# cestpasphoto/alpha-zero-general

Hardware: AMD Instinct MI355X
Metric: self-play env-steps/sec @ numMCTSSims=800, Splendor-2p (higher is better)
Workload: dtype f64

## Files before the change

alpha-zero-general_amd/csrc/game_splendor.hip.h:

```cpp
#pragma once
#include "azg_common.hip.h"
#include "splendor_tables.h"

namespace azg {

template <int NP>
struct SplendorDev {
    static constexpr bool STOCHASTIC = false;
    static constexpr bool RANDOM_SYM = false;
    static constexpr int P = NP;
    static constexpr int NN = NP + 1;
    static constexpr int ROWS = 32 + 10 * NP + NP * NP;
    static constexpr int COLS = 7;
    static constexpr int S = ROWS * COLS;
    static constexpr int SP = RoundUp16<S>::value;
    static constexpr int A = 81;
    static constexpr int AW = 2;
    static constexpr int R_NOBLES = 31, R_GEMS = 32 + NP, R_PNOB = 32 + 2 * NP, R_PCARDS = 32 + 3 * NP + NP * NP,
                         R_RES = 32 + 4 * NP + NP * NP;
    static constexpr int GOLD = 5, PTS = 6;
    static constexpr int MAX_MOVES = 62 * NP;

    __device__ static __forceinline__ const int8_t* row(const int8_t* st, int r) { return st + r * COLS; }
    __device__ static __forceinline__ int8_t* row(int8_t* st, int r) { return st + r * COLS; }
    __device__ static __forceinline__ int sum5(const int8_t* r) { return r[0] + r[1] + r[2] + r[3] + r[4]; }
    __device__ static __forceinline__ int sum7(const int8_t* r) { return sum5(r) + r[5] + r[6]; }

    __device__ static __forceinline__ int missing(const int8_t* cost, const int8_t* gems, const int8_t* cards) {
        int s = 0;
#pragma unroll
        for (int c = 0; c < 5; c++) {
            int8_t d = (int8_t)((int8_t)(cost[c] - gems[c]) - cards[c]);
            s += d > 0 ? d : 0;
        }
        return s;
    }

    __device__ static __forceinline__ void valid_mask(const int8_t* st, int player, uint64_t* mask_lds) {
        const int l = lane_id();
        const int8_t* bankp = row(st, 0);
        const int8_t* gemsp = row(st, R_GEMS + player);
        const int8_t* cardsp = row(st, R_PCARDS + player);
        const int8_t* lastres = row(st, R_RES + 6 * player + 5);
        int bank[5], gems[7], cards[5];
#pragma unroll
        for (int c = 0; c < 5; c++) { bank[c] = bankp[c]; cards[c] = cardsp[c]; }
#pragma unroll
        for (int c = 0; c < 7; c++) gems[c] = gemsp[c];
        const bool empty_slot = sum5(lastres) == 0;
        const int r = l < 12 ? 1 + 2 * l : l < 24 ? 1 + 2 * (l - 12) : l < 27 ? 25 + 2 * (l - 24)
                    : l < 30 ? R_RES + 6 * player + 2 * (l - 27) : 0;
        const int8_t* cr = row(st, r);
        int cost[5];
#pragma unroll
        for (int c = 0; c < 5; c++) cost[c] = cr[c];
        int gsum = 0;
#pragma unroll
        for (int c = 0; c < 7; c++) gsum += gems[c];
        int miss = 0, csum = 0;
#pragma unroll
        for (int c = 0; c < 5; c++) {
            const int8_t d = (int8_t)((int8_t)(cost[c] - gems[c]) - cards[c]);
            miss += d > 0 ? d : 0;
            csum += cost[c];
        }
        const bool nz = csum != 0;
        const bool ok_buy = miss <= gems[GOLD] && nz;
        const bool ok_res = empty_slot && nz;
        constexpr uint32_t g3[5] = SPL_GEMS3_COL_INIT, g2[5] = SPL_GEMS2_COL_INIT;
        const int i3 = (l - 30) & 31;
        const int ig = (l >= 60 ? l - 60 : l + 4) & 15;
        bool ok3 = true, okg = true;
        int k3 = 0;
#pragma unroll
        for (int c = 0; c < 5; c++) {
            const int t3 = (int)((g3[c] >> i3) & 1u), t2 = (int)((g2[c] >> ig) & 1u);
            ok3 = ok3 && ((int8_t)(bank[c] - t3) >= 0);
            okg = okg && ((int8_t)(gems[c] - t2) >= 0);
            k3 += t3;
        }
        ok3 = ok3 && (gsum + k3 <= 10);
        const int cs = l - 55, cg = l - 11;
        int bank_cs = bank[0], gems_cg = gems[0];
#pragma unroll
        for (int c = 1; c < 5; c++) { bank_cs = cs == c ? bank[c] : bank_cs; gems_cg = cg == c ? gems[c] : gems_cg; }
        const bool ok_same = bank_cs >= 4 && gsum + 2 <= 10;
        const bool v0 = l < 12 ? ok_buy : l < 27 ? ok_res : l < 30 ? ok_buy : l < 55 ? ok3 : l < 60 ? ok_same : okg;
        const bool v1 = l < 11 ? okg : l < 16 ? gems_cg >= 2 : l == 16;
        const uint64_t m0 = __ballot(v0);
        const uint64_t m1 = __ballot(v1);
        if (l == 0) { mask_lds[0] = m0; mask_lds[1] = m1; }
    }

    __device__ static bool get_deck_card(int8_t* st, int tier, long long seed, Rng& rng, int8_t* card14) {
        int8_t* cnt = row(st, 25 + 2 * tier);
        int8_t* bits = row(st, 26 + 2 * tier);
        int total = sum5(cnt);
        if (total == 0) return false;
        int color = 0, card_index = 0;
        if (seed == 0) {
            double u = rng.u01(), acc = 0.0;
            int k = 0;
            for (; k < 5; k++) { acc += (double)cnt[k] / (double)total; if (acc > u) break; }
            if (k >= 5) { for (k = 4; k > 0 && cnt[k] == 0; k--) {} }
            color = k;
            uint32_t b = (uint8_t)bits[color];
            int nb = __popc(b);
            double u2 = rng.u01();
            acc = 0.0;
            int idx = -1, last = 0;
            for (int i = 0; i < 8; i++) {
                int set = (b >> (7 - i)) & 1;
                if (set) last = i;
                acc += (double)set / (double)nb;
                if (acc > u2) { idx = i; break; }
            }
            card_index = idx < 0 ? last : idx;
        } else {
            int n = 0;
            long long seedv = 0, pw = 1;
            for (int c = 0; c < 5; c++) {
                uint32_t b = (uint8_t)bits[c];
                n += __popc(b);
                seedv += (long long)b * pw;
                pw *= 32;
            }
            long long x = 4594591LL * (seed + seedv);
            long long r = x % n;
            if (r < 0) r += n;
            int rem = (int)r;
            for (int c = 0; c < 5; c++) {
                uint32_t b = (uint8_t)bits[c];
                int pc = __popc(b);
                if (rem < pc) {
                    color = c;
                    for (int i = 0; i < 8; i++)
                        if ((b >> (7 - i)) & 1) { if (rem == 0) { card_index = i; break; } rem--; }
                    break;
                }
                rem -= pc;
            }
        }
        uint32_t b = (uint8_t)bits[color];
        b &= ~(0x80u >> card_index);
        bits[color] = (int8_t)(uint8_t)b;
        cnt[color] -= 1;
#pragma unroll
        for (int i = 0; i < 14; i++) card14[i] = SPL_CARDS[tier][color][card_index][i];
        return true;
    }

    __device__ static void fill_new_card(int8_t* st, int tier, int index, long long seed, Rng& rng) {
        int8_t* dst = row(st, 1 + 8 * tier + 2 * index);
        int8_t card[14];
        bool got = get_deck_card(st, tier, seed, rng, card);
#pragma unroll
        for (int i = 0; i < 14; i++) dst[i] = got ? card[i] : (int8_t)0;
    }

    static constexpr int SPW = SP / 4, NW = (SPW + 63) / 64;
    struct SW {
        uint32_t w[NW];
        __device__ __forceinline__ void load(const int8_t* st) {
#pragma unroll
            for (int k = 0; k < NW; k++) { const int i = lane_id() + 64 * k; w[k] = i < SPW ? ((const uint32_t*)st)[i] : 0u; }
        }
        __device__ __forceinline__ void store(int8_t* st) const {
#pragma unroll
            for (int k = 0; k < NW; k++) { const int i = lane_id() + 64 * k; if (i < SPW) ((uint32_t*)st)[i] = w[k]; }
        }
        __device__ __forceinline__ uint32_t rd(int d) const {
            uint32_t v = (uint32_t)__builtin_amdgcn_readlane((int)w[0], d & 63);
#pragma unroll
            for (int k = 1; k < NW; k++) {
                const uint32_t vk = (uint32_t)__builtin_amdgcn_readlane((int)w[k], d & 63);
                v = (d >> 6) == k ? vk : v;
            }
            return v;
        }
        __device__ __forceinline__ void wr(int d, uint32_t v) {
#pragma unroll
            for (int k = 0; k < NW; k++) w[k] = (lane_id() + 64 * k == d) ? v : w[k];
        }
        __device__ __forceinline__ uint64_t row(int r) const {
            const int o = 7 * r, d = o >> 2, sh = (o & 3) * 8;
            uint64_t v = (((uint64_t)rd(d + 1) << 32) | rd(d)) >> sh;
            if (sh > 8) v |= (uint64_t)rd(d + 2) << (64 - sh);
            return v & 0x00FFFFFFFFFFFFFFull;
        }
        __device__ __forceinline__ void set_row(int r, uint64_t v) {
            const int o = 7 * r, d = o >> 2, sh = (o & 3) * 8;
            const uint64_t m = 0x00FFFFFFFFFFFFFFull, M = m << sh, V = (v & m) << sh;
            wr(d, (rd(d) & ~(uint32_t)M) | (uint32_t)V);
            wr(d + 1, (rd(d + 1) & ~(uint32_t)(M >> 32)) | (uint32_t)(V >> 32));
            if (sh > 8) wr(d + 2, (rd(d + 2) & ~(uint32_t)(m >> (64 - sh))) | (uint32_t)((v & m) >> (64 - sh)));
        }
    };
    __device__ static __forceinline__ int B(uint64_t row, int c) { return (int)(int8_t)(uint8_t)(row >> (8 * c)); }
    __device__ static __forceinline__ int UB(uint64_t row, int c) { return (int)(uint8_t)(row >> (8 * c)); }
    __device__ static __forceinline__ void SETB(uint64_t& row, int c, int v) {
        row = (row & ~(0xFFull << (8 * c))) | ((uint64_t)(uint8_t)v << (8 * c));
    }
    __device__ static __forceinline__ int rsum5(uint64_t r) { return B(r, 0) + B(r, 1) + B(r, 2) + B(r, 3) + B(r, 4); }
    __device__ static __forceinline__ int rsum7(uint64_t r) { return rsum5(r) + B(r, 5) + B(r, 6); }

    __device__ static __forceinline__ uint32_t small_mod(uint32_t v, uint32_t n, float rn) {
        const uint32_t q = (uint32_t)((float)v * rn);
        int r = (int)(v - q * n);
        r = r < 0 ? r + (int)n : r;
        r = r >= (int)n ? r - (int)n : r;
        return (uint32_t)r;
    }
    __device__ static __forceinline__ int draw_mod(long long b, int n) {
        const float rn = 1.0f / (float)n;
        const bool neg = b < 0;
        const uint64_t ub = neg ? (uint64_t)(-b) : (uint64_t)b;
        uint32_t mb = 0;
#pragma unroll
        for (int k = 3; k >= 0; k--) mb = small_mod(mb * 65536u + (uint32_t)((ub >> (16 * k)) & 0xFFFFu), (uint32_t)n, rn);
        uint32_t ma = small_mod(70u, (uint32_t)n, rn);
        ma = small_mod(ma * 65536u + 7071u, (uint32_t)n, rn);
        uint32_t r = small_mod(ma * mb, (uint32_t)n, rn);
        if (neg && r) r = (uint32_t)n - r;
        return (int)r;
    }

    __device__ static __forceinline__ bool draw_card(SW& s, int tier, long long seed, Rng& rng, int* color_o, int* idx_o) {
        uint64_t cnt = s.row(25 + 2 * tier), bits = s.row(26 + 2 * tier);
        const int total = rsum5(cnt);
        if (total == 0) return false;
        int color = 0, card_index = 0;
        if (seed == 0) {
            const double u = rng.u01();
            double acc = 0.0;
            int k = 0;
            for (; k < 5; k++) { acc += (double)B(cnt, k) / (double)total; if (acc > u) break; }
            if (k >= 5) { for (k = 4; k > 0 && B(cnt, k) == 0; k--) {} }
            color = k;
            const uint32_t b = (uint32_t)UB(bits, color);
            const int nb = __popc(b);
            const double u2 = rng.u01();
            acc = 0.0;
            int idx = -1, last = 0;
            for (int i = 0; i < 8; i++) {
                const int set = (b >> (7 - i)) & 1;
                if (set) last = i;
                acc += (double)set / (double)nb;
                if (acc > u2) { idx = i; break; }
            }
            card_index = idx < 0 ? last : idx;
        } else {
            int n = 0;
            long long seedv = 0, pw = 1;
#pragma unroll
            for (int c = 0; c < 5; c++) {
                const uint32_t b = (uint32_t)UB(bits, c);
                n += __popc(b);
                seedv += (long long)b * pw;
                pw *= 32;
            }
            int rem = draw_mod(seed + seedv, n);
            for (int c = 0; c < 5; c++) {
                const uint32_t b = (uint32_t)UB(bits, c);
                const int pc = __popc(b);
                if (rem < pc) {
                    color = c;
                    for (int i = 0; i < 8; i++)
                        if ((b >> (7 - i)) & 1) { if (rem == 0) { card_index = i; break; } rem--; }
                    break;
                }
                rem -= pc;
            }
        }
        SETB(bits, color, (int)((uint32_t)UB(bits, color) & ~(0x80u >> card_index)));
        SETB(cnt, color, B(cnt, color) - 1);
        s.set_row(25 + 2 * tier, cnt);
        s.set_row(26 + 2 * tier, bits);
        *color_o = color; *idx_o = card_index;
        return true;
    }

    __device__ static __forceinline__ void buy_card(SW& s, uint64_t& bank, uint64_t& gems, uint64_t c0, uint64_t c1, int player) {
        uint64_t cards = s.row(R_PCARDS + player);
        int miss = 0;
#pragma unroll
        for (int c = 0; c < 5; c++) {
            const int8_t d = (int8_t)((int8_t)(B(c0, c) - B(gems, c)) - B(cards, c));
            miss += d > 0 ? d : 0;
        }
#pragma unroll
        for (int c = 0; c < 5; c++) {
            int8_t need = (int8_t)(B(c0, c) - B(cards, c));
            need = need < 0 ? (int8_t)0 : need;
            const int8_t g = (int8_t)B(gems, c);
            const int8_t paid = need < g ? need : g;
            SETB(gems, c, g - paid);
            SETB(bank, c, B(bank, c) + paid);
        }
        SETB(gems, GOLD, B(gems, GOLD) - miss);
        SETB(bank, GOLD, B(bank, GOLD) + miss);
#pragma unroll
        for (int c = 0; c < COLS; c++) SETB(cards, c, B(cards, c) + B(c1, c));
        s.set_row(R_PCARDS + player, cards);
        for (int i = 0; i < NN; i++) {
            const uint64_t noble = s.row(R_NOBLES + i);
            if (rsum5(noble) <= 0) continue;
            bool ok = true;
#pragma unroll
            for (int c = 0; c < 5; c++) ok = ok && B(cards, c) >= B(noble, c);
            if (ok) {
                s.set_row(R_PNOB + NN * player + i, noble);
                s.set_row(R_NOBLES + i, 0ull);
            }
        }
    }

    __device__ static __forceinline__ int gc_age(const int8_t* st) { return get_round(st); }

    __device__ static __forceinline__ bool move_uses_seed(int move) { return move < 27; }
    static constexpr int SEED_ACTIONS = 27;

    __device__ static int wave_make_move(int8_t* st, int move, int player, long long seed, Rng& rng) {
        move = uni_i32(move); player = uni_i32(player);
        seed = (long long)(((uint64_t)uni_u32((uint32_t)((uint64_t)seed >> 32)) << 32) | uni_u32((uint32_t)seed));
        const int l = lane_id();
        SW s;
        s.load(st);
        uint64_t bank = s.row(0), gems = s.row(R_GEMS + player);
        const int res = R_RES + 6 * player;
        int fill_row = -1, fill_tier = 0, fill_color = 0, fill_idx = 0;
        bool fill_got = false;
        int copy_src = -1, copy_dst = 0;
        int shift_i = -1;
        if (move < 12) {
            buy_card(s, bank, gems, s.row(1 + 2 * move), s.row(2 + 2 * move), player);
            fill_tier = move >> 2;
            fill_got = draw_card(s, fill_tier, seed, rng, &fill_color, &fill_idx);
            fill_row = 1 + 2 * move;
        } else if (move < 27) {
            const int i = move - 12;
            int slot = 2;
            for (int k = 2; k >= 0; k--) if (rsum5(s.row(res + 2 * k)) == 0) slot = k;
            if (i < 12) {
                copy_src = 1 + 2 * i; copy_dst = res + 2 * slot;
                fill_tier = i >> 2;
                fill_got = draw_card(s, fill_tier, seed, rng, &fill_color, &fill_idx);
                fill_row = 1 + 2 * i;
            } else {
                fill_tier = i - 12;
                fill_got = draw_card(s, fill_tier, seed, rng, &fill_color, &fill_idx);
                if (fill_got) fill_row = res + 2 * slot;
            }
            if (B(bank, GOLD) > 0 && rsum7(gems) <= 9) { SETB(gems, GOLD, B(gems, GOLD) + 1); SETB(bank, GOLD, B(bank, GOLD) - 1); }
        } else if (move < 30) {
            const int i = move - 27;
            buy_card(s, bank, gems, s.row(res + 2 * i), s.row(res + 2 * i + 1), player);
            shift_i = i;
        } else if (move < 80) {
            constexpr uint32_t g3[5] = SPL_GEMS3_COL_INIT, g2[5] = SPL_GEMS2_COL_INIT;
            const bool take = move < 60;
            const int i = take ? move - 30 : move - 60, nd = take ? 25 : 15;
#pragma unroll
            for (int c = 0; c < 5; c++) {
                const int k = i < nd ? (int)(((take ? g3[c] : g2[c]) >> (i & 31)) & 1u) : (c == i - nd ? 2 : 0);
                SETB(bank, c, take ? B(bank, c) - k : B(bank, c) + k);
                SETB(gems, c, take ? B(gems, c) + k : B(gems, c) - k);
            }
        }
        SETB(bank, PTS, B(bank, PTS) + 1);
        s.set_row(0, bank);
        s.set_row(R_GEMS + player, gems);
        s.store(st);
        wave_sync();
        if (copy_src >= 0 && l < 14) st[copy_dst * COLS + l] = st[copy_src * COLS + l];
        if (fill_row >= 0 && l < 14)
            st[fill_row * COLS + l] = fill_got ? SPL_CARDS[fill_tier][fill_color][fill_idx][l] : (int8_t)0;
        if (shift_i >= 0 && l < 6 * COLS) {
            const int lo = 2 * shift_i * COLS;
            const int8_t v = (l >= lo && l < 4 * COLS) ? st[res * COLS + l + 2 * COLS] : (int8_t)0;
            if (l >= lo) st[res * COLS + l] = v;
        }
        wave_sync();
        return (player + 1) % NP;
    }

    __device__ static __forceinline__ int get_round(const int8_t* st) { return (uint8_t)st[PTS]; }

    __device__ static int get_score(const int8_t* st, int p) {
        int s = row(st, R_PCARDS + p)[PTS];
#pragma unroll
        for (int i = 0; i < NN; i++) s += row(st, R_PNOB + NN * p + i)[PTS];
        return s;
    }

    __device__ static bool game_ended(const int8_t* st, int next_player, float* out , uint64_t* mask_scratch) {
        (void)next_player; (void)mask_scratch;
        int round = get_round(st);
#pragma unroll
        for (int p = 0; p < NP; p++) out[p] = 0.f;
        if (round % NP != 0) return false;
        float sc[NP];
        float mx = -1e30f;
#pragma unroll
        for (int p = 0; p < NP; p++) { sc[p] = (float)get_score(st, p); mx = sc[p] > mx ? sc[p] : mx; }
        if (!(mx >= 15.f || round >= MAX_MOVES)) return false;
        int cnt = 0;
#pragma unroll
        for (int p = 0; p < NP; p++) cnt += sc[p] == mx;
        bool several = cnt > 1;
        if (several) {
            mx = -1e30f;
#pragma unroll
            for (int p = 0; p < NP; p++) {
                int nb = sum5(row(st, R_PCARDS + p));
                sc[p] = (float)((double)sc[p] - (double)nb / 100.);
                mx = sc[p] > mx ? sc[p] : mx;
            }
            cnt = 0;
#pragma unroll
            for (int p = 0; p < NP; p++) cnt += sc[p] == mx;
            several = cnt > 1;
        }
#pragma unroll
        for (int p = 0; p < NP; p++) out[p] = (sc[p] == mx) ? (several ? 0.01f : 1.f) : -1.f;
        return true;
    }

    __device__ static void swap_players(int8_t* st, int8_t* tmp, int k) {
        for (int i = lane_id() + R_GEMS * COLS; i < S; i += 64) tmp[i] = st[i];
        wave_sync();
        for (int i = lane_id() + R_GEMS * COLS; i < S; i += 64) {
            int r = i / COLS, c = i - r * COLS, src;
            if (r < R_PNOB) src = R_GEMS + (r - R_GEMS + k) % NP;
            else if (r < R_PCARDS) src = R_PNOB + (r - R_PNOB + NN * k) % (NP * NN);
            else if (r < R_RES) src = R_PCARDS + (r - R_PCARDS + k) % NP;
            else src = R_RES + (r - R_RES + 6 * k) % (6 * NP);
            st[i] = tmp[src * COLS + c];
        }
        wave_sync();
    }

    static constexpr int NSYM_CAND = 10 + 2 * NP;
    __device__ static __forceinline__ int n_reserved(const int8_t* st, int pl) {
        int nb = 3;
        for (int c = 2; c >= 0; c--) if (sum5(row(st, R_RES + 6 * pl + 2 * c)) == 0) nb = c;
        return nb;
    }
    __device__ static __forceinline__ bool sym_exists(const int8_t* st, int c) {
        if (c < 10) return true;
        const int pl = (c - 10) >> 1, s = (c - 10) & 1;
        return SPL_RESERVE_SYM[n_reserved(st, pl)][s][0] >= 0;
    }
    __device__ static __forceinline__ int8_t sym_state_byte(const int8_t* st, int c, int i) {
        const int r = i / COLS, col = i - r * COLS;
        int src = r;
        if (c >= 1 && c < 10) {
            const int t = (c - 1) / 3, s = (c - 1) % 3, o = r - (1 + 8 * t);
            if (o >= 0 && o < 8) src = 1 + 8 * t + 2 * SPL_CARD_SYM[s][o >> 1] + (o & 1);
        } else if (c >= 10) {
            const int pl = (c - 10) >> 1, s = (c - 10) & 1, o = r - (R_RES + 6 * pl);
            if (o >= 0 && o < 6) src = R_RES + 6 * pl + 2 * SPL_RESERVE_SYM[n_reserved(st, pl)][s][o >> 1] + (o & 1);
        }
        return st[src * COLS + col];
    }
    __device__ static __forceinline__ int sym_action_src(const int8_t* st, int c, int a) {
        if (c >= 1 && c < 10) {
            const int t = (c - 1) / 3, s = (c - 1) % 3;
            if (a >= 4 * t && a < 4 * t + 4) return 4 * t + SPL_CARD_SYM[s][a - 4 * t];
            if (a >= 12 + 4 * t && a < 16 + 4 * t) return 12 + 4 * t + SPL_CARD_SYM[s][a - 12 - 4 * t];
        } else if (c >= 10 && ((c - 10) >> 1) == 0) {
            if (a >= 27 && a < 30) return 27 + SPL_RESERVE_SYM[n_reserved(st, 0)][(c - 10) & 1][a - 27];
        }
        return a;
    }

    __device__ static void init_board(int8_t* st, Rng& rng) {
        int8_t* bank = row(st, 0);
        const int gems_in_play = NP == 2 ? 4 : (NP == 3 ? 5 : 7);
        for (int c = 0; c < 5; c++) bank[c] = (int8_t)gems_in_play;
        bank[GOLD] = 5;
        for (int t = 0; t < 3; t++) {
            int len = SPL_DECK_LEN[t];
            for (int c = 0; c < 5; c++) {
                row(st, 25 + 2 * t)[c] = (int8_t)len;
                row(st, 26 + 2 * t)[c] = (int8_t)(uint8_t)(0xFF00u >> len);
            }
        }
        for (int t = 0; t < 3; t++)
            for (int i = 0; i < 4; i++) fill_new_card(st, t, i, 0, rng);
        int perm[10];
        for (int i = 0; i < 10; i++) perm[i] = i;
        for (int i = 0; i < NN; i++) {
            int j = i + (int)(rng.u01() * (10 - i));
            j = j > 9 ? 9 : j;
            int t = perm[i]; perm[i] = perm[j]; perm[j] = t;
            for (int c = 0; c < COLS; c++) row(st, 31 + i)[c] = SPL_NOBLES[perm[i]][c];
        }
    }
};

}
```

alpha-zero-general_amd/csrc/kernels.hip.h:

```cpp
#pragma once
#include <type_traits>
#include "forest.hip.h"

namespace azg {

template <class G>
__global__ __launch_bounds__(64) void k_env_valid_moves(const int8_t* states, const int32_t* players, int n,
                                                        uint8_t* out) {
    __shared__ __attribute__((aligned(16))) int8_t st[G::SP];
    __shared__ __attribute__((aligned(16))) uint64_t mask[G::AW];
    int t = blockIdx.x;
    if (t >= n) return;
    Forest<G>::load_state_unpadded(st, states + (size_t)t * G::S);
    G::valid_mask(st, players ? ld_agent_i32(players + t) : 0, mask);
    wave_sync();
    for (int a = lane_id(); a < G::A; a += 64) out[(size_t)t * G::A + a] = (uint8_t)((mask[a >> 6] >> (a & 63)) & 1);
}

template <class G>
__global__ __launch_bounds__(64) void k_env_next_state(const int8_t* states, const int32_t* players,
                                                       const int32_t* actions, const int64_t* seeds, int n,
                                                       int8_t* out_states, int32_t* out_next, uint64_t rng_seed,
                                                       uint64_t stream0, uint64_t* counters) {
    __shared__ __attribute__((aligned(16))) int8_t st[G::SP + MoveScratch<G>::value];
// ... 117 lines not shown
                                                        uint64_t* out_counters, int variant) {
    __shared__ __attribute__((aligned(16))) int8_t st[G::SP];
    int t = blockIdx.x;
    if (t >= n) return;
    for (int i = lane_id(); i < G::SP; i += 64) st[i] = 0;
    wave_sync();
    if (lane_id() == 0) {
        Rng rng{rng_seed, stream0 + (uint64_t)t, 0ull};
        if constexpr (InitTakesVariant<G>::value) G::init_board(st, rng, variant);
        else G::init_board(st, rng);
        if (out_counters) out_counters[t] = rng.counter;
    }
    wave_sync();
    Forest<G>::store_state_unpadded(out_states + (size_t)t * G::S, st);
}

template <class G>
__global__ __launch_bounds__(64) void k_forest_reset(ForestDev F) {
    int t = blockIdx.x;
    uint32_t* tab = Forest<G>::htab(F, t);
    for (int i = lane_id(); i < F.HT; i += 64) tab[i] = AZG_NONE;
    for (int i = lane_id(); i < Forest<G>::n_classes(F); i += 64) Forest<G>::rec_free(F, t)[i] = AZG_NONE;
    if (lane_id() == 0) {
        TreeHdr* H = &F.hdr[t];
        H->n_nodes = 0; H->heap_top = 0; H->root = AZG_NONE; H->root_rec = AZG_NONE; H->status = ST_IDLE;
        H->id_top = 0; H->n_free_ids = 0; H->free_units = 0;
        H->sim_idx = 0; H->n_sims = 0; H->pending_leaf = AZG_NONE; H->path_len = 0; H->mid_sim = 0;
    }
}

template <class G>
__device__ void begin_search_from_lds(const ForestDev& F, int t, TreeHdr& H, typename Forest<G>::Smem& sm, bool full) {
    using FR = Forest<G>;
    FR::store_state(F.root_state + (size_t)t * G::SP, sm.st);
    uint64_t h = FR::hash_state(sm.st);
    uint32_t free_slot;
    uint32_t found_rec = AZG_NONE;
    H.root = FR::probe(F, t, sm.st, h, &free_slot, &found_rec);
    H.root_rec = H.root == AZG_NONE ? AZG_NONE : found_rec;
    H.root_round = (uint32_t)G::gc_age(sm.st);
    H.is_full = full ? 1u : 0u;
    H.n_sims = (uint32_t)(full ? F.numMCTSSims : F.numMCTSSims / F.ratio_fullMCTS);
    H.forced = (full && F.forced_playouts) ? 1u : 0u;
    H.sim_idx = 0;
    H.status = ST_SEARCHING;
    H.pending_leaf = AZG_NONE;
    H.mid_sim = 0;
    H.noise_pending = (full && F.dirichletAlpha != 0.0 && H.root_rec != AZG_NONE) ? 1u : 0u;
}

template <class G>
__device__ __forceinline__ bool root_noise_tree(const ForestDev& F, int t, uint32_t root_rec, uint64_t c_sims,
                                                const double* root_noise, int noise_stride, float* dense ,
                                                uint64_t* mask ) {
    using FR = Forest<G>;
    const int l = lane_id();
    if (root_rec == AZG_NONE) return false;
    uint8_t* rec = FR::rec_ptr(F, t, root_rec);
    const RecHdr rh = load_uniform((const RecHdr*)rec);
    if (!(rh.flags & NF_EXPANDED)) return false;
    const int nv = rh.nv;

    const RecGeom RG = FR::geom(F);
    const RecIds ids(rec, RG);
    for (int i = l; i < G::A; i += 64) dense[i] = 0.f;
    if (l < G::AW) mask[l] = 0ull;
    wave_sync();
    for (int j = l; j < nv; j += 64) dense[ids[j]] = *(const float*)(rec + RG.hot((uint32_t)j) + AZG_H_P);
    if (l == 0)
        for (int j = 0; j < nv; j++) mask[ids[j] >> 6] |= 1ull << (ids[j] & 63);
    wave_sync();
    const double* nz = root_noise ? root_noise + (size_t)t * (noise_stride < 0 ? -noise_stride : noise_stride) : nullptr;
    FR::root_noise_dense(dense, mask, F.temp_root, nz, root_noise != nullptr && noise_stride < 0, F.dirichletAlpha,
                         mix64(mix64(forest_seed(F) ^ 0xA5A5A5A55A5A5A5AULL) + F.stream0 + (uint64_t)t), c_sims << 20);
    for (int j = l; j < nv; j += 64) *(float*)(rec + RG.hot((uint32_t)j) + AZG_H_P) = dense[ids[j]];
    return true;
}

template <class G>
__global__ __launch_bounds__(64) void k_root_noise(ForestDev F, const double* root_noise, int noise_stride) {
    __shared__ __attribute__((aligned(16))) float dense[G::A];
    __shared__ __attribute__((aligned(16))) uint64_t mask[G::AW];
    const int t = blockIdx.x;
    if (!ld_agent_u32(&F.hdr[t].noise_pending)) return;
    const uint32_t root_rec = ld_agent_u32(&F.hdr[t].root_rec);
    const uint64_t c_sims = ld_agent_u64(&F.hdr[t].c_sims);
    if (root_noise_tree<G>(F, t, root_rec, c_sims, root_noise, noise_stride, dense, mask) && lane_id() == 0)
        F.hdr[t].noise_pending = 0u;
}

__device__ __forceinline__ double ucb_score(float p, uint32_t n, double q, double cpuct, double sqrtNs, double sqrtNsEps,
                                            double fpu_init) {
    if (q != AZG_NANQ) return q + cpuct * (double)p * sqrtNs / (double)(1u + n);
    return fpu_init + cpuct * (double)p * sqrtNsEps;
}

template <class G, class = void> struct EndedFillsMask { static constexpr bool value = false; };
template <class G> struct EndedFillsMask<G, std::void_t<decltype(G::ENDED_FILLS_MASK)>> { static constexpr bool value = G::ENDED_FILLS_MASK; };

template <class G>
struct AsyncLeaf {
    static constexpr int MASK_OFF = G::SP;
    static constexpr int STRIDE = (G::SP + G::AW * 8 + 15) / 16 * 16;
};
template <class G, class HS, bool ASYNC = false>
__device__ __forceinline__ uint32_t create_leaf(const ForestDev& F, int t, HS& H, typename Forest<G>::Smem& sm,
                                             uint64_t h, uint32_t free_slot, int8_t* leaf_states, uint8_t* leaf_valid,
                                             bool* terminal, float* es, const typename Forest<G>::LeafPf* pf = nullptr) {
    using FR = Forest<G>;
    const int l = lane_id();
    const uint32_t id = FR::create_node(F, t, H, sm.st, h, free_slot, pf);
    if (id == AZG_NONE) return AZG_NONE;
    const bool ended = G::game_ended(sm.st, 0, es, sm.mask);
    int nv = 0;
    if (!ended) {
        if (!EndedFillsMask<G>::value) G::valid_mask(sm.st, 0, sm.mask);
        wave_sync();
#pragma unroll
        for (int k = 0; k < G::AW; k++) nv += __popcll(sm.mask[k]);
    }
    H.leaf_nv = (uint32_t)nv; H.leaf_node = id;
    int alloc_cls = 0;
    const uint32_t rec_off = FR::alloc_record(F, t, H, nv, id, &alloc_cls, pf);
    if (rec_off == AZG_NONE) return AZG_NONE;
    uint8_t* rec = FR::rec_ptr(F, t, rec_off);
    const uint8_t round = (uint8_t)G::gc_age(sm.st);
    if (l == 0) {
        RecHdr rh;
        rh.Ns = 0; rh.Qs = 0.f; rh.node_id = id; rh.nv = (uint16_t)nv; rh.flags = ended ? NF_TERMINAL : 0; rh.round = round;
#pragma unroll
        for (int p = 0; p < AZG_MAX_PLAYERS_DEV; p++) rh.Es[p] = (ended && p < G::P) ? es[p] : 0.f;
        if (G::P > AZG_MAX_PLAYERS_DEV && ended) rh.Qs = es[G::P > AZG_MAX_PLAYERS_DEV ? AZG_MAX_PLAYERS_DEV : 0];
        if (!ended) { rh.sq[0] = 0.0; rh.sq[1] = sqrt(0.0 + AZG_EPS); }
        *(RecHdr*)rec = rh;
        NodeHdr* nh = FR::nhdr(F, t, id);
        nh->rec_off = rec_off; nh->nv = (uint16_t)alloc_cls; nh->round = round; nh->flags = rh.flags;
    }
    *terminal = ended;
    if (!ended) {
        for (int a = l; a < G::A; a += 64) leaf_valid[(size_t)t * G::A + a] = (uint8_t)((sm.mask[a >> 6] >> (a & 63)) & 1);
        if constexpr (ASYNC) {
            using AL = AsyncLeaf<G>;
            static_assert(G::SP % 8 == 0, "8-byte granules");
            unsigned long long* dst = (unsigned long long*)(leaf_states + (size_t)t * AL::STRIDE);
            const unsigned long long* src = (const unsigned long long*)sm.st;
            for (int i = l; i < G::SP / 8 + G::AW; i += 64)
                __hip_atomic_store(dst + i, i < G::SP / 8 ? src[i] : (unsigned long long)sm.mask[i - G::SP / 8], __ATOMIC_RELAXED, __HIP_MEMORY_SCOPE_AGENT);
        } else
            FR::store_state_unpadded(leaf_states + (size_t)t * G::S, sm.st);
    }
    return rec_off;
}

template <class G, class HS, bool ASYNC = false>
__device__ __forceinline__ uint32_t resolve_edge(const ForestDev& F, int t, HS& H, typename Forest<G>::Smem& sm,
                                              uint32_t parent_node, int a, long long seed, int8_t* leaf_states,
                                              uint8_t* leaf_valid, bool* is_new, bool* terminal, float* es, Rng& rng,
                                              bool have_state = false, uint32_t st0 = 0, uint32_t st1 = 0, uint32_t st2 = 0) {
    using FR = Forest<G>;
#define AZG_SEG(k, d) H.cyc_seg[k] += (uint32_t)(d)
    long long c0 = AZG_CLK();
    typename FR::LeafPf pf = FR::leaf_pf_begin(F, t, H);
    if (have_state) {
        uint32_t* dst = (uint32_t*)sm.st;
        dst[lane_id()] = st0;
        if (lane_id() + 64 < FR::SPW) dst[lane_id() + 64] = st1;
        if (FR::SPW > 128 && lane_id() + 128 < FR::SPW) dst[lane_id() + 128] = st2;
        wave_sync();
    } else
        FR::load_state(sm.st, FR::nstate(F, t, parent_node));
    long long c1 = AZG_CLK(); AZG_SEG(0, c1 - c0);
    const int np = G::wave_make_move(sm.st, a, 0, seed, rng);
    c0 = AZG_CLK(); AZG_SEG(1, c0 - c1);
    FR::leaf_pf_links(F, t, pf);
    if (np != 0) G::swap_players(sm.st, sm.tmp, np);
    const uint64_t h = FR::hash_state(sm.st);
    c1 = AZG_CLK(); AZG_SEG(2, c1 - c0);
    uint32_t free_slot;
    uint32_t found_rec = AZG_NONE;
    const uint32_t found = FR::probe(F, t, sm.st, h, &free_slot, &found_rec);
    c0 = AZG_CLK(); AZG_SEG(3, c0 - c1);
    uint32_t crec;
    *is_new = false;
    if (found != AZG_NONE) crec = found_rec;
    else {
        const long long t_l = AZG_CLK();
        crec = create_leaf<G, HS, ASYNC>(F, t, H, sm, h, free_slot, leaf_states, leaf_valid, terminal, es, &pf);
        H.cyc_leaf += (uint32_t)(AZG_CLK() - t_l);
        if (crec == AZG_NONE) return AZG_NONE;
        *is_new = true;
    }
    return crec | ((uint32_t)np << AZG_CHILD_NP_SHIFT);
}

__device__ __forceinline__ void stat_add(uint64_t* p, uint64_t v) {
    __hip_atomic_fetch_add((unsigned long long*)p, (unsigned long long)v, __ATOMIC_RELAXED, __HIP_MEMORY_SCOPE_AGENT);
}

#ifdef AZG_CYC_COUNTERS
static __device__ unsigned long long g_prolog[16];
#define AZG_STAMP(k) do { long long c_; asm volatile("s_memtime %0\n\ts_waitcnt lgkmcnt(0)" : "=s"(c_)::"memory"); azg_stamp[k] = c_; } while (0)
#else
#define AZG_STAMP(k)
#endif

#ifndef AZG_PATH_PF
#define AZG_PATH_PF 16
#endif
template <class G>
struct ExpandIn {
    static constexpr int NA = (G::A + 63) / 64;
    uint32_t status, pending_leaf, path_len, leaf_is_root, sim_idx, is_full, pend_nv, pend_node;
    float pv[NA];
    uint8_t va[NA];
    float v[G::P];
    PathEnt pe0;
};

constexpr int AZG_HOT_WORDS = offsetof(TreeHdr, c_sims) / 4;
#define AZG_HW(w, field) ((w)[offsetof(TreeHdr, field) / 4])
template <bool HOT>
__device__ __forceinline__ void load_hot_header(const TreeHdr* Hp, uint32_t (&w)[AZG_HOT_WORDS]) {
    const uint32_t* p = (const uint32_t*)Hp;
#pragma unroll
    for (int i = 0; i < AZG_HOT_WORDS; i++) w[i] = HOT ? p[i] : __hip_atomic_load(p + i, __ATOMIC_RELAXED, __HIP_MEMORY_SCOPE_AGENT);
}
__device__ __forceinline__ void pin_hot_header(uint32_t (&w)[AZG_HOT_WORDS]) {
#pragma unroll
    for (int i = 0; i < AZG_HOT_WORDS; i++) { w[i] = uni_u32(w[i]); asm volatile("" : "+s"(w[i])); }
}

__device__ __forceinline__ void warm_kernarg_448() {
    const auto ka = __builtin_amdgcn_kernarg_segment_ptr();
    uint32_t a, b, c, d, e, f, g;
    asm volatile("s_load_dword %0, %7, 0x0\n\ts_load_dword %1, %7, 0x40\n\ts_load_dword %2, %7, 0x80\n\t"
                 "s_load_dword %3, %7, 0xc0\n\ts_load_dword %4, %7, 0x100\n\ts_load_dword %5, %7, 0x140\n\t"
                 "s_load_dword %6, %7, 0x180\n\ts_waitcnt lgkmcnt(0)"
                 : "=&s"(a), "=&s"(b), "=&s"(c), "=&s"(d), "=&s"(e), "=&s"(f), "=&s"(g)
                 : "s"(ka)
                 : "memory");
}

template <class G, bool ASYNC = false>
__device__ __forceinline__ void expand_load(const ForestDev& F, int t, const float* pi, const float* vin,
                                            const uint8_t* leaf_valid, ExpandIn<G>& in, const uint32_t (&hw)[AZG_HOT_WORDS]) {
    const int l = lane_id();
    (void)hw;
#pragma unroll
    for (int k = 0; k < ExpandIn<G>::NA; k++) {
        const int a = l + 64 * k;
        if constexpr (ASYNC)
            in.pv[k] = a < G::A ? __uint_as_float(__hip_atomic_load((const uint32_t*)pi + (size_t)t * G::A + a, __ATOMIC_RELAXED, __HIP_MEMORY_SCOPE_AGENT)) : 0.f;
        else
        in.pv[k] = a < G::A ? pi[(size_t)t * G::A + a] : 0.f;
        in.va[k] = a < G::A ? leaf_valid[(size_t)t * G::A + a] : (uint8_t)0;
    }
#pragma unroll
    for (int p = 0; p < G::P; p++)
        in.v[p] = __uint_as_float(__hip_atomic_load((const uint32_t*)vin + (size_t)t * G::P + p, __ATOMIC_RELAXED, __HIP_MEMORY_SCOPE_AGENT));
    in.pe0 = l < AZG_PATH_PF ? (F.path + (size_t)t * AZG_MAXD)[l] : PathEnt{0u, 0, 0, 0};
}

template <class G>
__device__ __forceinline__ void expand_header(ExpandIn<G>& in, const uint32_t (&hw)[AZG_HOT_WORDS]) {
    in.status = AZG_HW(hw, status); in.pending_leaf = AZG_HW(hw, pending_leaf); in.path_len = AZG_HW(hw, path_len);
    in.leaf_is_root = AZG_HW(hw, leaf_is_root); in.sim_idx = AZG_HW(hw, sim_idx); in.is_full = AZG_HW(hw, is_full);
    in.pend_nv = AZG_HW(hw, pending_nv); in.pend_node = AZG_HW(hw, pending_node);
}

template <class G>
__device__ __forceinline__ bool expand_apply(const ForestDev& F, int t, const ExpandIn<G>& in, float* dense ,
                                             PathEnt* path , int noise_enabled, long long* azg_stamp) {
    using FR = Forest<G>;
    constexpr int NA = ExpandIn<G>::NA;
    const int l = lane_id();
    TreeHdr* Hp = &F.hdr[t];
    const int depth = (int)uni_u32(in.path_len);
    const int nv = (int)uni_u32(in.pend_nv);
    const uint32_t sim = uni_u32(in.sim_idx);
    uint8_t* rec = FR::rec_ptr(F, t, uni_u32(in.pending_leaf));
    RecHdr* rhp = (RecHdr*)rec;
    const RecGeom RG = FR::geom(F);
    const PathEnt* gp = F.path + (size_t)t * AZG_MAXD;
    if (l < AZG_PATH_PF) path[l] = in.pe0;
    for (int d = l + AZG_PATH_PF; d < depth; d += 64) path[d] = gp[d];
    constexpr bool SUM_IN_REGS = G::A >= 8 && G::A <= 256;
    if (!SUM_IN_REGS) {
#pragma unroll
        for (int k = 0; k < NA; k++) if (l + 64 * k < G::A) dense[l + 64 * k] = in.pv[k];
    }
    wave_sync();
    const bool dir_now = (noise_enabled && uni_u32(in.leaf_is_root) && sim == 0 && uni_u32(in.is_full) && F.dirichletAlpha != 0.0);
    float s = 1.f;
    if (!dir_now) {
        if constexpr (SUM_IN_REGS) s = np_sum_regs<G::A>(in.pv);
        else s = np_sum_f32_static<G::A>(dense);
    }
    AZG_STAMP(2);
    int base_rank = 0;
#pragma unroll
    for (int k = 0; k < NA; k++) {
        const uint64_t m = __ballot(in.va[k] != 0);
        if (in.va[k]) {
            const uint32_t j = (uint32_t)(base_rank + __popcll(m & ((1ull << l) - 1ull)));
            uint4 e0;
            e0.x = __float_as_uint(dir_now ? in.pv[k] : in.pv[k] / s); e0.y = 0u;
            e0.z = (uint32_t)__double_as_longlong(AZG_NANQ); e0.w = (uint32_t)((uint64_t)__double_as_longlong(AZG_NANQ) >> 32);
            *(uint4*)(rec + RG.hot(j)) = e0;
            const int nu = (j % RG.PC) < RG.SE ? F.U : 1;
            for (int u = 0; u < nu; u++) *(uint32_t*)(rec + RG.child(j, (uint32_t)u)) = AZG_NONE;
            if (FR::IDB == 1) *(uint8_t*)(rec + RG.id(j)) = (uint8_t)(l + 64 * k);
            else *(uint16_t*)(rec + RG.id(j)) = (uint16_t)(l + 64 * k);
        }
        base_rank += __popcll(m);
    }
    if (l == 0) {
        rhp->Ns = 0; rhp->Qs = in.v[0]; rhp->flags = NF_EXPANDED;
        FR::nhdr(F, t, uni_u32(in.pend_node))->flags = NF_EXPANDED;
    }
    AZG_STAMP(3);
    FR::backup(F, t, path, depth, in.v);
    AZG_STAMP(4);
    if (l == 0) {
        Hp->sim_idx = sim + 1;
        Hp->status = ST_SEARCHING;
// ... 492 lines not shown
```

Before: 83950.

## Use SWAR byte arithmetic and register-passed state in Splendor move step

Replaces per-byte extract/insert loops in Splendor's card buying, gem moves and card drawing with SWAR packed-byte add/sub/min/compare helpers, a constexpr gem-move table, and table-driven reciprocal modular reduction. The make-move entry now takes the parent state directly from per-lane registers loaded from global memory, skipping the shared-memory staging load. swap_players gathers through registers with closed-form source indexing instead of a tmp-buffer copy and modulo arithmetic. The aim is fewer ALU instructions and LDS round-trips per expansion step, at the cost of subtle correctness risk in the SWAR sign and overflow handling and in the reciprocal tables.

New measurement: 46710. -44.4%, worse.

```diff
diff --git a/alpha-zero-general_amd/csrc/game_splendor.hip.h b/alpha-zero-general_amd/csrc/game_splendor.hip.h
--- a/alpha-zero-general_amd/csrc/game_splendor.hip.h
+++ b/alpha-zero-general_amd/csrc/game_splendor.hip.h
@@ -1,8 +1,32 @@
 #pragma once
 #include "azg_common.hip.h"
 #include "splendor_tables.h"
+#include "splendor_swar.h"
 
 namespace azg {
+
+AZG_TABLE_QUAL static const uint32_t SPL_RECIP[41] = SPL_RECIP_INIT;
+AZG_TABLE_QUAL static const uint32_t SPL_MULT[41] = SPL_MULT_INIT;
+
+struct SplGemMoves { uint64_t v[50]; };
+constexpr SplGemMoves spl_gem_moves() {
+    constexpr uint32_t g3[5] = SPL_GEMS3_COL_INIT, g2[5] = SPL_GEMS2_COL_INIT;
+    SplGemMoves t{};
+    for (int i = 0; i < 50; i++) {
+        uint64_t k = 0;
+        for (int c = 0; c < 5; c++) {
+            uint64_t b = 0;
+            if (i < 25) b = (g3[c] >> i) & 1u;
+            else if (i < 30) b = c == i - 25 ? 2u : 0u;
+            else if (i < 45) b = (g2[c] >> (i - 30)) & 1u;
+            else b = c == i - 45 ? 2u : 0u;
+            k |= b << (8 * c);
+        }
+        t.v[i] = k;
+    }
+    return t;
+}
+AZG_TABLE_QUAL static const SplGemMoves SPL_GEM_MOVES = spl_gem_moves();
 
 template <int NP>
 struct SplendorDev {
@@ -196,34 +220,10 @@
             if (sh > 8) wr(d + 2, (rd(d + 2) & ~(uint32_t)(m >> (64 - sh))) | (uint32_t)((v & m) >> (64 - sh)));
         }
     };
-    __device__ static __forceinline__ int B(uint64_t row, int c) { return (int)(int8_t)(uint8_t)(row >> (8 * c)); }
-    __device__ static __forceinline__ int UB(uint64_t row, int c) { return (int)(uint8_t)(row >> (8 * c)); }
-    __device__ static __forceinline__ void SETB(uint64_t& row, int c, int v) {
-        row = (row & ~(0xFFull << (8 * c))) | ((uint64_t)(uint8_t)v << (8 * c));
-    }
-    __device__ static __forceinline__ int rsum5(uint64_t r) { return B(r, 0) + B(r, 1) + B(r, 2) + B(r, 3) + B(r, 4); }
-    __device__ static __forceinline__ int rsum7(uint64_t r) { return rsum5(r) + B(r, 5) + B(r, 6); }
-
-    __device__ static __forceinline__ uint32_t small_mod(uint32_t v, uint32_t n, float rn) {
-        const uint32_t q = (uint32_t)((float)v * rn);
-        int r = (int)(v - q * n);
-        r = r < 0 ? r + (int)n : r;
-        r = r >= (int)n ? r - (int)n : r;
-        return (uint32_t)r;
-    }
-    __device__ static __forceinline__ int draw_mod(long long b, int n) {
-        const float rn = 1.0f / (float)n;
-        const bool neg = b < 0;
-        const uint64_t ub = neg ? (uint64_t)(-b) : (uint64_t)b;
-        uint32_t mb = 0;
-#pragma unroll
-        for (int k = 3; k >= 0; k--) mb = small_mod(mb * 65536u + (uint32_t)((ub >> (16 * k)) & 0xFFFFu), (uint32_t)n, rn);
-        uint32_t ma = small_mod(70u, (uint32_t)n, rn);
-        ma = small_mod(ma * 65536u + 7071u, (uint32_t)n, rn);
-        uint32_t r = small_mod(ma * mb, (uint32_t)n, rn);
-        if (neg && r) r = (uint32_t)n - r;
-        return (int)r;
-    }
+    __device__ static __forceinline__ int B(uint64_t row, int c) { return swar::byte_s8(row, c); }
+    __device__ static __forceinline__ int rsum5(uint64_t r) { return swar::sum5_s8(r); }
+    __device__ static __forceinline__ int rsum7(uint64_t r) { return swar::sum7_s8(r); }
+    static constexpr uint64_t ONE_GOLD = 1ull << (8 * GOLD), ONE_PTS = 1ull << (8 * PTS);
 
     __device__ static __forceinline__ bool draw_card(SW& s, int tier, long long seed, Rng& rng, int* color_o, int* idx_o) {
         uint64_t cnt = s.row(25 + 2 * tier), bits = s.row(26 + 2 * tier);
@@ -237,7 +237,7 @@
             for (; k < 5; k++) { acc += (double)B(cnt, k) / (double)total; if (acc > u) break; }
             if (k >= 5) { for (k = 4; k > 0 && B(cnt, k) == 0; k--) {} }
             color = k;
-            const uint32_t b = (uint32_t)UB(bits, color);
+            const uint32_t b = (uint32_t)(uint8_t)(bits >> (8 * color));
             const int nb = __popc(b);
             const double u2 = rng.u01();
             acc = 0.0;
@@ -250,18 +250,14 @@
             }
             card_index = idx < 0 ? last : idx;
         } else {
-            int n = 0;
-            long long seedv = 0, pw = 1;
-#pragma unroll
+            const int n = __popcll(bits & swar::L5);
+            const uint32_t rn = SPL_RECIP[n], ma = SPL_MULT[n];
+            long long seedv = 0;
+#pragma unroll
+            for (int c = 0; c < 5; c++) seedv += (long long)((bits >> (8 * c)) & 0xFFull) << (5 * c);
+            int rem = spl_draw_mod(seed + seedv, n, rn, ma);
             for (int c = 0; c < 5; c++) {
-                const uint32_t b = (uint32_t)UB(bits, c);
-                n += __popc(b);
-                seedv += (long long)b * pw;
-                pw *= 32;
-            }
-            int rem = draw_mod(seed + seedv, n);
-            for (int c = 0; c < 5; c++) {
-                const uint32_t b = (uint32_t)UB(bits, c);
+                const uint32_t b = (uint32_t)(uint8_t)(bits >> (8 * c));
                 const int pc = __popc(b);
                 if (rem < pc) {
                     color = c;
@@ -272,8 +268,8 @@
                 rem -= pc;
             }
         }
-        SETB(bits, color, (int)((uint32_t)UB(bits, color) & ~(0x80u >> card_index)));
-        SETB(cnt, color, B(cnt, color) - 1);
+        bits &= ~((uint64_t)(0x80u >> card_index) << (8 * color));
+        cnt = swar::sub8(cnt, 1ull << (8 * color));
         s.set_row(25 + 2 * tier, cnt);
         s.set_row(26 + 2 * tier, bits);
         *color_o = color; *idx_o = card_index;
@@ -281,34 +277,20 @@
     }
 
     __device__ static __forceinline__ void buy_card(SW& s, uint64_t& bank, uint64_t& gems, uint64_t c0, uint64_t c1, int player) {
+        using namespace swar;
         uint64_t cards = s.row(R_PCARDS + player);
-        int miss = 0;
-#pragma unroll
-        for (int c = 0; c < 5; c++) {
-            const int8_t d = (int8_t)((int8_t)(B(c0, c) - B(gems, c)) - B(cards, c));
-            miss += d > 0 ? d : 0;
-        }
-#pragma unroll
-        for (int c = 0; c < 5; c++) {
-            int8_t need = (int8_t)(B(c0, c) - B(cards, c));
-            need = need < 0 ? (int8_t)0 : need;
-            const int8_t g = (int8_t)B(gems, c);
-            const int8_t paid = need < g ? need : g;
-            SETB(gems, c, g - paid);
-            SETB(bank, c, B(bank, c) + paid);
-        }
-        SETB(gems, GOLD, B(gems, GOLD) - miss);
-        SETB(bank, GOLD, B(bank, GOLD) + miss);
-#pragma unroll
-        for (int c = 0; c < COLS; c++) SETB(cards, c, B(cards, c) + B(c1, c));
+        const int miss = sum5_s8(relu8(sub8(sub8(c0, gems), cards)));
+        const uint64_t need = relu8(sub8(c0, cards));
+        const uint64_t paid = min8_nonneg_a(need, gems) & L5;
+        const uint64_t gold = (uint64_t)(uint8_t)miss << (8 * GOLD);
+        gems = sub8(sub8(gems, paid), gold);
+        bank = add8(add8(bank, paid), gold);
+        cards = add8(cards, c1) & L7;
         s.set_row(R_PCARDS + player, cards);
         for (int i = 0; i < NN; i++) {
             const uint64_t noble = s.row(R_NOBLES + i);
             if (rsum5(noble) <= 0) continue;
-            bool ok = true;
-#pragma unroll
-            for (int c = 0; c < 5; c++) ok = ok && B(cards, c) >= B(noble, c);
-            if (ok) {
+            if ((ge8_signed(cards, noble) & (H8 & L5)) == (H8 & L5)) {
                 s.set_row(R_PNOB + NN * player + i, noble);
                 s.set_row(R_NOBLES + i, 0ull);
             }
@@ -321,11 +303,22 @@
     static constexpr int SEED_ACTIONS = 27;
 
     __device__ static int wave_make_move(int8_t* st, int move, int player, long long seed, Rng& rng) {
+        SW s;
+        s.load(st);
+        return step_regs(st, s, move, player, seed, rng);
+    }
+    __device__ static __forceinline__ int wave_make_move_regs(int8_t* st, uint32_t w0, uint32_t w1, uint32_t w2, int move, int player,
+                                                              long long seed, Rng& rng) {
+        SW s;
+        s.w[0] = w0;
+        if (NW > 1) s.w[1] = w1;
+        if (NW > 2) s.w[NW > 2 ? 2 : 0] = w2;
+        return step_regs(st, s, move, player, seed, rng);
+    }
+    __device__ static __forceinline__ int step_regs(int8_t* st, SW& s, int move, int player, long long seed, Rng& rng) {
         move = uni_i32(move); player = uni_i32(player);
         seed = (long long)(((uint64_t)uni_u32((uint32_t)((uint64_t)seed >> 32)) << 32) | uni_u32((uint32_t)seed));
         const int l = lane_id();
-        SW s;
-        s.load(st);
         uint64_t bank = s.row(0), gems = s.row(R_GEMS + player);
         const int res = R_RES + 6 * player;
         int fill_row = -1, fill_tier = 0, fill_color = 0, fill_idx = 0;
@@ -351,23 +344,17 @@
                 fill_got = draw_card(s, fill_tier, seed, rng, &fill_color, &fill_idx);
                 if (fill_got) fill_row = res + 2 * slot;
             }
-            if (B(bank, GOLD) > 0 && rsum7(gems) <= 9) { SETB(gems, GOLD, B(gems, GOLD) + 1); SETB(bank, GOLD, B(bank, GOLD) - 1); }
+            if (B(bank, GOLD) > 0 && rsum7(gems) <= 9) { gems = swar::add8(gems, ONE_GOLD); bank = swar::sub8(bank, ONE_GOLD); }
         } else if (move < 30) {
             const int i = move - 27;
             buy_card(s, bank, gems, s.row(res + 2 * i), s.row(res + 2 * i + 1), player);
             shift_i = i;
         } else if (move < 80) {
-            constexpr uint32_t g3[5] = SPL_GEMS3_COL_INIT, g2[5] = SPL_GEMS2_COL_INIT;
-            const bool take = move < 60;
-            const int i = take ? move - 30 : move - 60, nd = take ? 25 : 15;
-#pragma unroll
-            for (int c = 0; c < 5; c++) {
-                const int k = i < nd ? (int)(((take ? g3[c] : g2[c]) >> (i & 31)) & 1u) : (c == i - nd ? 2 : 0);
-                SETB(bank, c, take ? B(bank, c) - k : B(bank, c) + k);
-                SETB(gems, c, take ? B(gems, c) + k : B(gems, c) - k);
-            }
-        }
-        SETB(bank, PTS, B(bank, PTS) + 1);
+            const uint64_t k = SPL_GEM_MOVES.v[move - 30];
+            if (move < 60) { bank = swar::sub8(bank, k); gems = swar::add8(gems, k); }
+            else { bank = swar::add8(bank, k); gems = swar::sub8(gems, k); }
+        }
+        bank = swar::add8(bank, ONE_PTS);
         s.set_row(0, bank);
         s.set_row(R_GEMS + player, gems);
         s.store(st);
@@ -426,17 +413,22 @@
         return true;
     }
 
+    __device__ static __forceinline__ int swap_src(int i, int k) {
+        constexpr int B_PNOB = R_PNOB * COLS, B_PCARDS = R_PCARDS * COLS, B_RES = R_RES * COLS;
+        const int L = (i < B_PNOB ? 1 : i < B_PCARDS ? NN : i < B_RES ? 1 : 6) * COLS;
+        const int end = i < B_PNOB ? B_PNOB : i < B_PCARDS ? B_PCARDS : i < B_RES ? B_RES : S;
+        const int src = i + (NP == 2 ? L : k * L);
+        return src >= end ? src - NP * L : src;
+    }
     __device__ static void swap_players(int8_t* st, int8_t* tmp, int k) {
-        for (int i = lane_id() + R_GEMS * COLS; i < S; i += 64) tmp[i] = st[i];
+        (void)tmp;
+        constexpr int B0 = R_GEMS * COLS, NIT = (S - B0 + 63) / 64;
+        int8_t v[NIT];
+#pragma unroll
+        for (int j = 0; j < NIT; j++) { const int i = lane_id() + B0 + 64 * j; v[j] = i < S ? st[swap_src(i, k)] : (int8_t)0; }
         wave_sync();
-        for (int i = lane_id() + R_GEMS * COLS; i < S; i += 64) {
-            int r = i / COLS, c = i - r * COLS, src;
-            if (r < R_PNOB) src = R_GEMS + (r - R_GEMS + k) % NP;
-            else if (r < R_PCARDS) src = R_PNOB + (r - R_PNOB + NN * k) % (NP * NN);
-            else if (r < R_RES) src = R_PCARDS + (r - R_PCARDS + k) % NP;
-            else src = R_RES + (r - R_RES + 6 * k) % (6 * NP);
-            st[i] = tmp[src * COLS + c];
-        }
+#pragma unroll
+        for (int j = 0; j < NIT; j++) { const int i = lane_id() + B0 + 64 * j; if (i < S) st[i] = v[j]; }
         wave_sync();
     }
 
diff --git a/alpha-zero-general_amd/csrc/kernels.hip.h b/alpha-zero-general_amd/csrc/kernels.hip.h
--- a/alpha-zero-general_amd/csrc/kernels.hip.h
+++ b/alpha-zero-general_amd/csrc/kernels.hip.h
@@ -293,6 +293,9 @@
     return rec_off;
 }
 
+template <class G, class = void> struct MakeMoveTakesRegs { static constexpr bool value = false; };
+template <class G> struct MakeMoveTakesRegs<G, std::void_t<decltype(&G::wave_make_move_regs)>> { static constexpr bool value = true; };
+
 template <class G, class HS, bool ASYNC = false>
 __device__ __forceinline__ uint32_t resolve_edge(const ForestDev& F, int t, HS& H, typename Forest<G>::Smem& sm,
                                               uint32_t parent_node, int a, long long seed, int8_t* leaf_states,
@@ -302,7 +305,15 @@
 #define AZG_SEG(k, d) H.cyc_seg[k] += (uint32_t)(d)
     long long c0 = AZG_CLK();
     typename FR::LeafPf pf = FR::leaf_pf_begin(F, t, H);
-    if (have_state) {
+    if constexpr (MakeMoveTakesRegs<G>::value) {
+        static_assert(FR::SPW <= 192, "three dwords per lane");
+        if (!have_state) {
+            const uint32_t* nsp = (const uint32_t*)FR::nstate(F, t, parent_node);
+            st0 = nsp[lane_id()];
+            st1 = lane_id() + 64 < FR::SPW ? nsp[lane_id() + 64] : 0u;
+            st2 = (FR::SPW > 128 && lane_id() + 128 < FR::SPW) ? nsp[lane_id() + 128] : 0u;
+        }
+    } else if (have_state) {
         uint32_t* dst = (uint32_t*)sm.st;
         dst[lane_id()] = st0;
         if (lane_id() + 64 < FR::SPW) dst[lane_id() + 64] = st1;
@@ -311,7 +322,9 @@
     } else
         FR::load_state(sm.st, FR::nstate(F, t, parent_node));
     long long c1 = AZG_CLK(); AZG_SEG(0, c1 - c0);
-    const int np = G::wave_make_move(sm.st, a, 0, seed, rng);
+    int np;
+    if constexpr (MakeMoveTakesRegs<G>::value) np = G::wave_make_move_regs(sm.st, st0, st1, st2, a, 0, seed, rng);
+    else np = G::wave_make_move(sm.st, a, 0, seed, rng);
     c0 = AZG_CLK(); AZG_SEG(1, c0 - c1);
     FR::leaf_pf_links(F, t, pf);
     if (np != 0) G::swap_players(sm.st, sm.tmp, np);
diff --git a/alpha-zero-general_amd/csrc/splendor_swar.h b/alpha-zero-general_amd/csrc/splendor_swar.h
--- /dev/null
+++ b/alpha-zero-general_amd/csrc/splendor_swar.h
@@ -0,0 +1,60 @@
+#pragma once
+#include <stdint.h>
+#if defined(__HIPCC__)
+#define AZG_HD __host__ __device__ __forceinline__
+#else
+#define AZG_HD inline
+#endif
+
+namespace azg {
+namespace swar {
+
+constexpr uint64_t H8 = 0x8080808080808080ull;
+constexpr uint64_t L5 = 0x000000FFFFFFFFFFull;
+constexpr uint64_t L7 = 0x00FFFFFFFFFFFFFFull;
+
+AZG_HD uint64_t add8(uint64_t a, uint64_t b) { return ((a & ~H8) + (b & ~H8)) ^ ((a ^ b) & H8); }
+AZG_HD uint64_t sub8(uint64_t a, uint64_t b) { return ((a | H8) - (b & ~H8)) ^ ((a ^ ~b) & H8); }
+AZG_HD uint64_t neg_mask8(uint64_t x) { const uint64_t s = x & H8; return (s << 1) - (s >> 7); }
+AZG_HD uint64_t relu8(uint64_t x) { return x & ~neg_mask8(x); }
+AZG_HD uint64_t min8_nonneg_a(uint64_t a, uint64_t b) {
+    const uint64_t lt = neg_mask8(sub8(a, b) & ~b);
+    return (a & lt) | (b & ~lt);
+}
+AZG_HD uint64_t ge8_signed(uint64_t a, uint64_t b) {
+    const uint64_t ua = a ^ H8, ub = b ^ H8;
+    const uint64_t t = (ua | H8) - (ub & ~H8);
+    return ((ua & ~ub) | (~(ua ^ ub) & t)) & H8;
+}
+AZG_HD int sum5_s8(uint64_t x) {
+    x &= L5;
+    const uint64_t e = (x & 0x00FF00FF00FF00FFull) + ((x >> 8) & 0x00FF00FF00FF00FFull);
+    const uint32_t f = (uint32_t)e + (uint32_t)(e >> 32);
+    return (int)((f + (f >> 16)) & 0xFFFFu) - 256 * __builtin_popcountll(x & H8);
+}
+AZG_HD int byte_s8(uint64_t row, int c) { return (int)(int8_t)(uint8_t)(row >> (8 * c)); }
+AZG_HD int sum7_s8(uint64_t x) { return sum5_s8(x) + byte_s8(x, 5) + byte_s8(x, 6); }
+
+}
+
+#define SPL_RECIP_INIT {0u, 0u, 2147483649u, 1431655766u, 1073741825u, 858993460u, 715827883u, 613566757u, 536870913u, 477218589u, \
+    429496730u, 390451573u, 357913942u, 330382100u, 306783379u, 286331154u, 268435457u, 252645136u, 238609295u, 226050911u, 214748365u, \
+    204522253u, 195225787u, 186737709u, 178956971u, 171798692u, 165191050u, 159072863u, 153391690u, 148102321u, 143165577u, 138547333u, \
+    134217729u, 130150525u, 126322568u, 122713352u, 119304648u, 116080198u, 113025456u, 110127367u, 107374183u}
+#define SPL_MULT_INIT {0, 0, 1, 1, 3, 1, 1, 1, 7, 1, 1, 1, 7, 1, 1, 1, 15, 1, 1, 11, 11, 1, 1, 19, 7, 16, 1, 1, 15, 5, 1, 19, 31, 1, 1, 1, 19, 5, 11, 1, 31}
+
+AZG_HD uint32_t spl_mulhi_u32(uint32_t a, uint32_t b) { return (uint32_t)(((uint64_t)a * (uint64_t)b) >> 32); }
+AZG_HD uint32_t spl_small_mod(uint32_t v, uint32_t n, uint32_t rn) { return n == 1u ? 0u : v - spl_mulhi_u32(v, rn) * n; }
+AZG_HD int spl_draw_mod(long long b, int n, uint32_t rn, uint32_t ma) {
+    const bool neg = b < 0;
+    const uint64_t ub = neg ? (uint64_t)0 - (uint64_t)b : (uint64_t)b;
+    const uint32_t un = (uint32_t)n;
+    uint32_t mb = spl_small_mod((uint32_t)(ub >> 42), un, rn);
+    mb = spl_small_mod((mb << 21) | (uint32_t)((ub >> 21) & 0x1FFFFFu), un, rn);
+    mb = spl_small_mod((mb << 21) | (uint32_t)(ub & 0x1FFFFFu), un, rn);
+    uint32_t r = spl_small_mod(ma * mb, un, rn);
+    if (neg && r) r = un - r;
+    return (int)r;
+}
+
+}
```
